# NEUROINFORMATICS-GROUP-FAV-KIV-ZCU/EEG_DataAnalysisPackage

Measured on AMD Instinct MI355X. Metric: epochs/sec feature-extracted (whole node) + % HBM roofline, 1/2/4/8 GPUs, higher is better.
Workload: dtype f64

## Files before the change

eeg_dataanalysispackage_amd/csrc/launch.h:

```cpp
#pragma once

#include <hip/hip_runtime_api.h>

#include <cstdint>

#include "guard.h"

namespace eegfx {

constexpr int kMaxChannels = 64;

struct ChanSel {
  int32_t col[kMaxChannels];
  float res[kMaxChannels];
};

hipError_t launch_cut_epochs(hipStream_t st, const void* raw, int fmt, int64_t n_frames, int ct,
                             const ChanSel& sel, int C, const int64_t* pos, int64_t n,
                             double* out, void* scratch, int* err);
hipError_t launch_cut_epochs(hipStream_t st, const void* raw, int fmt, int64_t n_frames, int ct,
                             const ChanSel& sel, int C, const int64_t* pos, int64_t n,
                             float* out, void* scratch, int* err);
bool cut_features_supported(int fmt, int ct, int C, const void* raw, const double* out,
                            const double* feat);
hipError_t launch_cut_features(hipStream_t st, const void* raw, int fmt, int64_t n_frames, int ct,
                               const ChanSel& sel, int C, const int64_t* pos, int64_t n,
                               double* out, double* feat, bool fast, void* scratch, int* err,
                               const Guard& guard);
bool cut_features_supported(int fmt, int ct, int C, const void* raw, const float* out,
                            const double* feat);
hipError_t launch_cut_features(hipStream_t st, const void* raw, int fmt, int64_t n_frames, int ct,
                               const ChanSel& sel, int C, const int64_t* pos, int64_t n,
                               float* out, double* feat, bool fast, void* scratch, int* err,
                               const Guard& guard);
hipError_t launch_features_from_epochs(hipStream_t st, const double* ep, int64_t n, int C, int skip,
                                       int nfeat, bool fast, double* out, int row_stride,
                                       const Guard& guard);
hipError_t launch_features_from_epochs(hipStream_t st, const float* ep, int64_t n, int C, int skip,
                                       int nfeat, bool fast, double* out, int row_stride,
                                       const Guard& guard);
hipError_t launch_narrow_epochs(hipStream_t st, const double* in, float* out, int64_t count);
bool features_small_supported(int C);
struct MailboxCmd {
  uint64_t req;
  uint32_t done;
  uint32_t stop;
  uint32_t alive;
  uint32_t pad_;
  const double* rows;
  double* out;
};
inline uint64_t mailbox_request(uint32_t seq, int C, int nfeat, int64_t n) {
  return (uint64_t)seq << 32 | (uint64_t)(C - 1) << 26 | (uint64_t)(nfeat - 1) << 21 |
         (uint64_t)n;
}
hipError_t launch_features_mailbox(hipStream_t st, MailboxCmd* mb, uint64_t idle_ticks,
                                   uint32_t gen);
hipError_t launch_features_small(hipStream_t st, const double* rows, int64_t n, int C, int nfeat,
                                 double* out);
hipError_t launch_synth(hipStream_t st, int16_t* dst, int64_t n_frames, int ct, uint64_t seed);

bool streaming_reads(int64_t n_frames, int64_t n, int64_t min_spacing);

bool fused_supported(int fmt, int ct, int C, const double* out);
size_t fused_scratch_bytes(int64_t n, int C);
hipError_t launch_fused_baseline(hipStream_t st, const void* raw, int64_t n_frames, int ct,
                                 const ChanSel& sel, int C, const int64_t* pos, int64_t n,
                                 void* scratch, int* err, int* guard_count,
                                 const Guard* guard = nullptr);
hipError_t launch_fused_window(hipStream_t st, const void* raw, int64_t n_frames, int ct,
                               const ChanSel& sel, int C, const int64_t* pos, int64_t n, bool fast,
                               const void* scratch, double* out, const Guard& guard,
                               bool track = false);
int64_t fused_window_bytes_per_epoch(int ct, int C);

bool wide_supported(int fmt, int ct, int C);
bool baseline_any_supported(int fmt, int ct, int C);
hipError_t launch_baseline_any(hipStream_t st, const void* raw, int fmt, int64_t n_frames, int ct,
                               const ChanSel& sel, int C, const int64_t* pos, int64_t n,
                               void* scratch, int* err, int* guard_count,
                               const Guard* guard = nullptr);
hipError_t launch_window_wide(hipStream_t st, const void* raw, int fmt, int64_t n_frames, int ct,
                              const ChanSel& sel, int C, const int64_t* pos, int64_t n, bool fast,
                              const void* scratch, double* out, const Guard& guard,
                              bool track = false);

hipError_t launch_pyramid_from_epochs(hipStream_t st, const double* ep, int64_t n, int C, int skip,
                                      int nfeat, double* out, int row_stride);
hipError_t launch_pyramid_from_epochs(hipStream_t st, const float* ep, int64_t n, int C, int skip,
                                      int nfeat, double* out, int row_stride);

hipError_t launch_guard_fixup_raw(hipStream_t st, const void* raw, int fmt, int64_t n_frames,
                                  int ct, const ChanSel& sel, int C, const int64_t* pos,
                                  const void* scratch, const Guard& g, double* out);

struct LrState {
  int32_t iter;
  int32_t converged;
  int32_t updates;
  int32_t pad;
  double w[];
};
constexpr int kLrMaxFeatures = 1024;

struct PlanResult {
  int64_t selected;
  int64_t balance;
  int64_t first_unparsable;
};
size_t plan_scratch_bytes(int64_t n);
hipError_t launch_plan_markers(hipStream_t st, const int64_t* pos, const int32_t* stim, int64_t n,
                               int64_t n_frames, int32_t guessed, int d0, void* scratch,
                               int64_t* pos_out, double* label_out, PlanResult* result);
int lr_grid(int64_t n);
hipError_t launch_lr_validate(hipStream_t st, const double* y, int64_t n, LrState* state);
constexpr int kGradLogistic = 0;
constexpr int kGradHinge = 1;
hipError_t launch_lr_iteration(hipStream_t st, int grad, const double* X, const double* y,
                               int64_t n, int d, const uint32_t* mask, int64_t count,
                               LrState* state, double* partial, int G, double step_size,
                               double reg, double tol, int max_iter);
hipError_t launch_lr_predict(hipStream_t st, int grad, const double* X, int64_t n, int d,
                             const double* w, double intercept, double threshold,
                             int use_threshold, double* out);


struct DtDecision {
  int32_t feature;
  int32_t split;
  int32_t left, right;
};
struct DtNode {
  int32_t feature, left, right, pad;
  double threshold, predict;
};
constexpr int kDtMaxBins = 256;
constexpr int kDtLdsCounters = 32768;
hipError_t launch_dt_bin(hipStream_t st, const double* X, const double* y, int64_t n, int d,
                         int T, const int32_t* nthr, const double* thr, int32_t* flags,
                         uint8_t* bins, uint8_t* label, int32_t* slot);
hipError_t launch_dt_hist(hipStream_t st, const uint8_t* bins, const uint8_t* label,
                          const int32_t* slot, int64_t n, int d, int B, int g0, int g,
                          uint32_t* hist);
hipError_t launch_dt_route(hipStream_t st, const uint8_t* bins, int64_t n, int d,
                           const DtDecision* dec, int32_t* slot);
hipError_t launch_dt_gather(hipStream_t st, const double* X, int d, const int64_t* idx, int64_t m,
                            double* out);
hipError_t launch_dt_predict(hipStream_t st, const double* X, int64_t n, int d,
                             const DtNode* nodes, int n_nodes, double* out);

hipError_t launch_rf_init(hipStream_t st, const uint8_t* weight, int64_t n, int num_trees,
                          int32_t* slot);
hipError_t launch_rf_hist(hipStream_t st, const uint8_t* bins, const uint8_t* label,
                          const uint8_t* weight, const int32_t* slot, int64_t n, int d, int B,
                          int k, int s0, int g, const int32_t* trees, int nt, const int32_t* sub,
                          uint32_t* hist);
hipError_t launch_rf_route(hipStream_t st, const uint8_t* bins, int64_t n, int d,
                           const int32_t* trees, int nt, int s0, int g, const DtDecision* dec,
                           int32_t* slot);
hipError_t launch_rf_predict(hipStream_t st, const double* X, int64_t n, int d,
                             const DtNode* nodes, const int32_t* offsets, int num_trees,
                             double* out);

}
```

eeg_dataanalysispackage_amd/csrc/logreg.hip:

```cpp
#include <hip/hip_runtime.h>

#include <cstdint>
#include <cstdlib>

#include "launch.h"

namespace eegfx {
namespace dev {

constexpr int kLrWaves = 4;
#ifndef EEGFX_LR_UNROLL
#define EEGFX_LR_UNROLL 4
#endif

__device__ __forceinline__ double wave_sum(double v) {
#pragma unroll
  for (int off = 32; off > 0; off >>= 1) v += __shfl_xor(v, off, 64);
  return v;
}

template <int GRAD>
__device__ __forceinline__ double grad_mult(double margin, double y) {
  if constexpr (GRAD == 0) {
    return 1.0 / (1.0 + exp(-margin)) - y;
  } else {
    const double s = 2.0 * y - 1.0;
    return 1.0 > s * margin ? -s : 0.0;
  }
}

template <int GRAD>
__device__ __forceinline__ double axpy_row(double mult, double x, double acc) {
  if constexpr (GRAD == 0) {
    return __builtin_fma(mult, x, acc);
  } else {
    return mult != 0.0 ? __builtin_fma(mult, x, acc) : acc;
  }
}

__device__ __forceinline__ bool sampled(const uint32_t* __restrict__ mask, int64_t r) {
  return !mask || ((mask[r >> 5] >> (r & 31)) & 1u);
}

template <int KD, int GRAD>
__global__ __launch_bounds__(64 * kLrWaves) void lr_grad_kernel(
    const double* __restrict__ X, const double* __restrict__ y, int64_t n, int d,
    const uint32_t* __restrict__ mask, const LrState* __restrict__ st,
    double* __restrict__ partial) {
  if (st->converged) return;
  __shared__ double acc_s[kLrWaves][64 * KD];
  const int lane = threadIdx.x & 63, w = threadIdx.x >> 6;
  const double* wt = st->w;
  double wv[KD], acc[KD];
#pragma unroll
  for (int k = 0; k < KD; ++k) {
    const int f = lane + 64 * k;
    wv[k] = f < d ? wt[f] : 0.0;
    acc[k] = 0.0;
  }
  const int64_t stride = (int64_t)gridDim.x * kLrWaves;
  for (int64_t r = (int64_t)blockIdx.x * kLrWaves + w; r < n; r += stride) {
    if (!sampled(mask, r)) continue;
    const double* row = X + r * d;
    double x[KD];
    double dot = 0.0;
#pragma unroll
    for (int k = 0; k < KD; ++k) {
      const int f = lane + 64 * k;
      x[k] = f < d ? row[f] : 0.0;
      dot = __builtin_fma(x[k], wv[k], dot);
    }
    dot = wave_sum(dot);
    const double mult = grad_mult<GRAD>(dot, y[r]);
#pragma unroll
    for (int k = 0; k < KD; ++k) acc[k] = axpy_row<GRAD>(mult, x[k], acc[k]);
  }
#pragma unroll
  for (int k = 0; k < KD; ++k) acc_s[w][lane + 64 * k] = acc[k];
  __syncthreads();
  for (int f = threadIdx.x; f < d; f += blockDim.x) {
    double s = acc_s[0][f];
#pragma unroll
    for (int v = 1; v < kLrWaves; ++v) s += acc_s[v][f];
    partial[(int64_t)blockIdx.x * d + f] = s;
  }
}

template <int CTRL>
__device__ __forceinline__ double dpp_d(double v) {
  const uint64_t u = __builtin_bit_cast(uint64_t, v);
  const int lo = __builtin_amdgcn_update_dpp(0, (int)(uint32_t)u, CTRL, 0xF, 0xF, false);
  const int hi = __builtin_amdgcn_update_dpp(0, (int)(uint32_t)(u >> 32), CTRL, 0xF, 0xF, false);
  return __builtin_bit_cast(double, ((uint64_t)(uint32_t)hi << 32) | (uint32_t)lo);
}
__device__ __forceinline__ double row16_sum(double v) {
  v += dpp_d<0xB1>(v);
  v += dpp_d<0x4E>(v);
  v += dpp_d<0x141>(v);
  v += dpp_d<0x140>(v);
  return v;
}

template <int FPL, int GRAD>
__global__ __launch_bounds__(64 * kLrWaves) void lr_grad16_kernel(
    const double* __restrict__ X, const double* __restrict__ y, int64_t n, int d,
    const uint32_t* __restrict__ mask, const LrState* __restrict__ st,
    double* __restrict__ partial) {
  if (st->converged) return;
  __shared__ double acc_s[kLrWaves * 4][16 * FPL];
  const int lane = threadIdx.x & 63, w = threadIdx.x >> 6;
  const int q = lane >> 4, j = lane & 15;
  double wv[FPL], acc[FPL];
#pragma unroll
  for (int k = 0; k < FPL; ++k) {
    const int f = j + 16 * k;
    wv[k] = f < d ? st->w[f] : 0.0;
    acc[k] = 0.0;
  }
  constexpr int U = EEGFX_LR_UNROLL;
  const int64_t stride = (int64_t)gridDim.x * kLrWaves * 4 * U;
  for (int64_t r0 = ((int64_t)blockIdx.x * kLrWaves + w) * 4 * U; r0 < n; r0 += stride) {
    double x[U][FPL], dot[U], yy[U];
#pragma unroll
    for (int u = 0; u < U; ++u) {
      const int64_t r = r0 + 4 * u + q;
      dot[u] = 0.0;
      if constexpr (GRAD == 0) {
        const bool ok = r < n && sampled(mask, r);
        const double* row = X + (ok ? r : 0) * d;
#pragma unroll
        for (int k = 0; k < FPL; ++k) {
          const int f = j + 16 * k;
          x[u][k] = (ok && f < d) ? row[f] : 0.0;
          dot[u] = __builtin_fma(x[u][k], wv[k], dot[u]);
        }
        yy[u] = ok ? y[r] : 0.0;
      } else {
        const double* row = X + (r < n ? r : n - 1) * d;
#pragma unroll
        for (int k = 0; k < FPL; ++k) {
          const int f = j + 16 * k;
          x[u][k] = row[f < d ? f : d - 1];
          dot[u] = __builtin_fma(x[u][k], wv[k], dot[u]);
        }
        yy[u] = y[r < n ? r : n - 1];
      }
    }
    double mult[U], msum = 0.0;
#pragma unroll
    for (int u = 0; u < U; ++u) {
      const double m = row16_sum(dot[u]);
      const bool ok = r0 + 4 * u + q < n && sampled(mask, r0 + 4 * u + q);
      mult[u] = ok ? grad_mult<GRAD>(m, yy[u]) : 0.0;
      msum += m;
    }
    if constexpr (GRAD == 1) {
      if (__builtin_amdgcn_ballot_w64(!(__builtin_fabs(msum) <= __DBL_MAX__)) != 0) {
#pragma unroll
        for (int u = 0; u < U; ++u) {
          double dt = 0.0;
#pragma unroll
          for (int k = 0; k < FPL; ++k) {
            if (j + 16 * k >= d) x[u][k] = 0.0;
            dt = __builtin_fma(x[u][k], wv[k], dt);
          }
          const double m = row16_sum(dt);
          const bool ok = r0 + 4 * u + q < n && sampled(mask, r0 + 4 * u + q);
          const double mu = ok ? grad_mult<GRAD>(m, yy[u]) : 0.0;
#pragma unroll
          for (int k = 0; k < FPL; ++k) acc[k] = axpy_row<GRAD>(mu, x[u][k], acc[k]);
        }
        continue;
      }
    }
#pragma unroll
    for (int u = 0; u < U; ++u) {
#pragma unroll
      for (int k = 0; k < FPL; ++k) acc[k] = __builtin_fma(mult[u], x[u][k], acc[k]);
    }
  }
#pragma unroll
  for (int k = 0; k < FPL; ++k) acc_s[w * 4 + q][j + 16 * k] = acc[k];
  __syncthreads();
  for (int f = threadIdx.x; f < d; f += blockDim.x) {
    double s = acc_s[0][f];
#pragma unroll
    for (int v = 1; v < kLrWaves * 4; ++v) s += acc_s[v][f];
    partial[(int64_t)blockIdx.x * d + f] = s;
  }
}

__global__ __launch_bounds__(256) void lr_update_kernel(const double* __restrict__ partial, int G,
                                                        int64_t n, int d, double step_size,
                                                        double reg, double tol, int max_iter,
                                                        LrState* __restrict__ st) {
  if (st->converged) return;
  __shared__ double red[2][256];
  __shared__ double gs[256];
  const int it = st->iter + 1;
  const double step = step_size / sqrt((double)it);
  const int K = d <= 128 ? (int)blockDim.x / d : 1;
  if (K > 1) {
    const int t = threadIdx.x, jj = t / d, f = t - jj * d;
    if (jj < K) {
      double a0 = 0.0, a1 = 0.0;
      int b = jj;
      for (; b + K < G; b += 2 * K) {
        a0 += partial[(int64_t)b * d + f];
        a1 += partial[(int64_t)(b + K) * d + f];
      }
      if (b < G) a0 += partial[(int64_t)b * d + f];
      gs[t] = a0 + a1;
    }
    __syncthreads();
  }
  double diff2 = 0.0, norm2 = 0.0;
  for (int f = threadIdx.x; f < d; f += blockDim.x) {
    double g = 0.0;
    if (K > 1) {
      for (int jj = 0; jj < K; ++jj) g += gs[jj * d + f];
    } else {
      for (int b = 0; b < G; ++b) g += partial[(int64_t)b * d + f];
    }
    g = g / (double)n;
    const double old = st->w[f];
    double nw = old * (1.0 - step * reg);
    nw = nw + (-step) * g;
    st->w[f] = nw;
    diff2 += (old - nw) * (old - nw);
    norm2 += nw * nw;
  }
  red[0][threadIdx.x] = diff2;
  red[1][threadIdx.x] = norm2;
  __syncthreads();
  for (int s = 128; s > 0; s >>= 1) {
    if ((int)threadIdx.x < s) {
      red[0][threadIdx.x] += red[0][threadIdx.x + s];
      red[1][threadIdx.x] += red[1][threadIdx.x + s];
    }
    __syncthreads();
  }
  if (threadIdx.x == 0) {
    st->iter = it;
    const int up = st->updates + 1;
    st->updates = up;
    const double diff = sqrt(red[0][0]), nrm = sqrt(red[1][0]);
    if ((up >= 2 && diff < tol * (nrm > 1.0 ? nrm : 1.0)) || it >= max_iter) st->converged = 1;
  }
}

__global__ void lr_skip_kernel(int max_iter, LrState* __restrict__ st) {
  if (st->converged || threadIdx.x != 0) return;
  st->iter += 1;
  if (st->iter >= max_iter) st->converged = 1;
}

template <int KD, int KIND>
__global__ __launch_bounds__(256) void lr_predict_kernel(const double* __restrict__ X, int64_t n,
                                                         int d, const double* __restrict__ wt,
                                                         double intercept, double threshold,
                                                         int use_threshold,
                                                         double* __restrict__ out) {
  const int lane = threadIdx.x & 63;
  const int64_t r = (int64_t)blockIdx.x * 4 + (threadIdx.x >> 6);
  if (r >= n) return;
  double dot = 0.0;
#pragma unroll
  for (int k = 0; k < KD; ++k) {
    const int f = lane + 64 * k;
    if (f < d) dot = __builtin_fma(X[r * d + f], wt[f], dot);
  }
  dot = wave_sum(dot);
  if (lane == 0) {
    const double margin = dot + intercept;
    const double score = KIND == 0 ? 1.0 / (1.0 + exp(-margin)) : margin;
    out[r] = use_threshold ? (score > threshold ? 1.0 : 0.0) : score;
  }
}

__global__ __launch_bounds__(256) void lr_validate_kernel(const double* __restrict__ y, int64_t n,
                                                          LrState* __restrict__ st) {
  for (int64_t i = (int64_t)blockIdx.x * blockDim.x + threadIdx.x; i < n;
       i += (int64_t)gridDim.x * blockDim.x)
    if (!(y[i] == 0.0 || y[i] == 1.0)) st->converged = 2;
}

}

hipError_t launch_lr_validate(hipStream_t st, const double* y, int64_t n, LrState* state) {
  const int64_t g = (n + 255) / 256;
  hipLaunchKernelGGL(dev::lr_validate_kernel, dim3((unsigned)(g < 1 ? 1 : (g > 4096 ? 4096 : g))),
                     dim3(256), 0, st, y, n, state);
  return hipGetLastError();
}

int lr_grid(int64_t n) {
  constexpr int64_t cap = 512;
  const int64_t g = (n + 16 * dev::kLrWaves - 1) / (16 * dev::kLrWaves);
  return (int)(g < 1 ? 1 : (g > cap ? cap : g));
}

#define EEGFX_LR_KD(KD, CALL) \
  case KD:                    \
    CALL;                     \
    break;

template <int GRAD>
static hipError_t lr_iteration(hipStream_t st, const double* X, const double* y, int64_t n, int d,
                               const uint32_t* mask, int64_t count, LrState* state,
                               double* partial, int G, double step_size, double reg, double tol,
                               int max_iter) {
  if (count == 0) {
    hipLaunchKernelGGL(dev::lr_skip_kernel, dim3(1), dim3(64), 0, st, max_iter, state);
    return hipGetLastError();
  }
  if (d <= 128) {
    const int fpl = (d + 15) / 16;
    switch (fpl <= 1 ? 1 : fpl <= 2 ? 2 : fpl <= 3 ? 3 : fpl <= 4 ? 4 : 8) {
      EEGFX_LR_KD(1, hipLaunchKernelGGL((dev::lr_grad16_kernel<1, GRAD>), dim3(G), dim3(256), 0,
                                        st, X, y, n, d, mask, state, partial))
      EEGFX_LR_KD(2, hipLaunchKernelGGL((dev::lr_grad16_kernel<2, GRAD>), dim3(G), dim3(256), 0,
                                        st, X, y, n, d, mask, state, partial))
      EEGFX_LR_KD(3, hipLaunchKernelGGL((dev::lr_grad16_kernel<3, GRAD>), dim3(G), dim3(256), 0,
                                        st, X, y, n, d, mask, state, partial))
      EEGFX_LR_KD(4, hipLaunchKernelGGL((dev::lr_grad16_kernel<4, GRAD>), dim3(G), dim3(256), 0,
                                        st, X, y, n, d, mask, state, partial))
      EEGFX_LR_KD(8, hipLaunchKernelGGL((dev::lr_grad16_kernel<8, GRAD>), dim3(G), dim3(256), 0,
                                        st, X, y, n, d, mask, state, partial))
    }
  } else {
    const int kd = (d + 63) / 64;
    switch (kd <= 1 ? 1 : kd <= 2 ? 2 : kd <= 4 ? 4 : kd <= 8 ? 8 : 16) {
      EEGFX_LR_KD(1, hipLaunchKernelGGL((dev::lr_grad_kernel<1, GRAD>), dim3(G), dim3(256), 0, st,
                                        X, y, n, d, mask, state, partial))
      EEGFX_LR_KD(2, hipLaunchKernelGGL((dev::lr_grad_kernel<2, GRAD>), dim3(G), dim3(256), 0, st,
                                        X, y, n, d, mask, state, partial))
      EEGFX_LR_KD(4, hipLaunchKernelGGL((dev::lr_grad_kernel<4, GRAD>), dim3(G), dim3(256), 0, st,
                                        X, y, n, d, mask, state, partial))
      EEGFX_LR_KD(8, hipLaunchKernelGGL((dev::lr_grad_kernel<8, GRAD>), dim3(G), dim3(256), 0, st,
                                        X, y, n, d, mask, state, partial))
      EEGFX_LR_KD(16, hipLaunchKernelGGL((dev::lr_grad_kernel<16, GRAD>), dim3(G), dim3(256), 0,
                                         st, X, y, n, d, mask, state, partial))
    }
  }
  hipLaunchKernelGGL(dev::lr_update_kernel, dim3(1), dim3(256), 0, st, partial, G, count, d,
                     step_size, reg, tol, max_iter, state);
  return hipGetLastError();
}

hipError_t launch_lr_iteration(hipStream_t st, int grad, const double* X, const double* y,
                               int64_t n, int d, const uint32_t* mask, int64_t count,
                               LrState* state, double* partial, int G, double step_size,
                               double reg, double tol, int max_iter) {
  return grad == kGradHinge ? lr_iteration<1>(st, X, y, n, d, mask, count, state, partial, G,
                                              step_size, reg, tol, max_iter)
                            : lr_iteration<0>(st, X, y, n, d, mask, count, state, partial, G,
                                              step_size, reg, tol, max_iter);
}

template <int KIND>
static hipError_t lr_predict(hipStream_t st, const double* X, int64_t n, int d, const double* w,
                             double intercept, double threshold, int use_threshold, double* out) {
  const dim3 grid((unsigned)((n + 3) / 4));
  const int kd = (d + 63) / 64;
  switch (kd <= 1 ? 1 : kd <= 2 ? 2 : kd <= 4 ? 4 : kd <= 8 ? 8 : 16) {
    EEGFX_LR_KD(1, hipLaunchKernelGGL((dev::lr_predict_kernel<1, KIND>), grid, dim3(256), 0, st, X,
                                      n, d, w, intercept, threshold, use_threshold, out))
    EEGFX_LR_KD(2, hipLaunchKernelGGL((dev::lr_predict_kernel<2, KIND>), grid, dim3(256), 0, st, X,
                                      n, d, w, intercept, threshold, use_threshold, out))
    EEGFX_LR_KD(4, hipLaunchKernelGGL((dev::lr_predict_kernel<4, KIND>), grid, dim3(256), 0, st, X,
                                      n, d, w, intercept, threshold, use_threshold, out))
    EEGFX_LR_KD(8, hipLaunchKernelGGL((dev::lr_predict_kernel<8, KIND>), grid, dim3(256), 0, st, X,
                                      n, d, w, intercept, threshold, use_threshold, out))
    EEGFX_LR_KD(16, hipLaunchKernelGGL((dev::lr_predict_kernel<16, KIND>), grid, dim3(256), 0, st,
                                       X, n, d, w, intercept, threshold, use_threshold, out))
  }
  return hipGetLastError();
}

hipError_t launch_lr_predict(hipStream_t st, int grad, const double* X, int64_t n, int d,
                             const double* w, double intercept, double threshold,
                             int use_threshold, double* out) {
  if (n == 0) return hipSuccess;
  return grad == kGradHinge
             ? lr_predict<1>(st, X, n, d, w, intercept, threshold, use_threshold, out)
             : lr_predict<0>(st, X, n, d, w, intercept, threshold, use_threshold, out);
}
#undef EEGFX_LR_KD

}
```

eeg_dataanalysispackage_amd/csrc/lds_dma.h:

```cpp
#pragma once

#include <hip/hip_runtime.h>

#include <cstdint>

namespace eegfx {
namespace dev {

typedef __attribute__((address_space(3))) void* lds_ptr_t;

#ifndef EEGFX_DMA_POLICY
#define EEGFX_DMA_POLICY ""
#endif

template <bool NT = false>
__device__ __forceinline__ void dma16_s(const uint8_t* sbase, uint32_t voff, const void* lds_dst) {
  const uint32_t lds = (uint32_t)(uintptr_t)(lds_ptr_t)lds_dst;
  uint32_t saved;
  if constexpr (NT) {
    asm volatile(
        "s_mov_b32 %0, m0\n\t"
        "s_mov_b32 m0, %1\n\t"
        "s_nop 0\n\t"
        "global_load_lds_dwordx4 %2, %3 nt\n\t"
        "s_nop 0\n\t"
        "s_mov_b32 m0, %0"
        : "=&s"(saved)
        : "s"(lds), "v"(voff), "s"(sbase)
        : "memory");
  } else {
    asm volatile(
        "s_mov_b32 %0, m0\n\t"
        "s_mov_b32 m0, %1\n\t"
        "s_nop 0\n\t"
        "global_load_lds_dwordx4 %2, %3" EEGFX_DMA_POLICY "\n\t"
        "s_nop 0\n\t"
        "s_mov_b32 m0, %0"
        : "=&s"(saved)
        : "s"(lds), "v"(voff), "s"(sbase)
        : "memory");
  }
}

__device__ __forceinline__ void dma_drain() { asm volatile("s_waitcnt vmcnt(0)" ::: "memory"); }

}
}
```

Before: 1.189 billion.

## Fuse logistic-regression update into gradient kernel via last-block-arrives ticket

Removes the separate single-block lr_update_kernel launch per iteration. Each gradient block now stores its partial sum atomically and takes a ticket on a counter in LrState, and the last block to arrive performs the reduction and weight update. The partial reduction loop is also batched so more loads are in flight. This saves one kernel launch and one dependency per iteration, at the cost of device-scope atomics and fences, and it requires the repurposed pad field to start at zero.

```diff
diff --git a/eeg_dataanalysispackage_amd/csrc/launch.h b/eeg_dataanalysispackage_amd/csrc/launch.h
--- a/eeg_dataanalysispackage_amd/csrc/launch.h
+++ b/eeg_dataanalysispackage_amd/csrc/launch.h
@@ -98,7 +98,7 @@
   int32_t iter;
   int32_t converged;
   int32_t updates;
-  int32_t pad;
+  int32_t arrived;
   double w[];
 };
 constexpr int kLrMaxFeatures = 1024;
diff --git a/eeg_dataanalysispackage_amd/csrc/logreg.hip b/eeg_dataanalysispackage_amd/csrc/logreg.hip
--- a/eeg_dataanalysispackage_amd/csrc/logreg.hip
+++ b/eeg_dataanalysispackage_amd/csrc/logreg.hip
@@ -42,159 +42,34 @@
   return !mask || ((mask[r >> 5] >> (r & 31)) & 1u);
 }
 
-template <int KD, int GRAD>
-__global__ __launch_bounds__(64 * kLrWaves) void lr_grad_kernel(
-    const double* __restrict__ X, const double* __restrict__ y, int64_t n, int d,
-    const uint32_t* __restrict__ mask, const LrState* __restrict__ st,
-    double* __restrict__ partial) {
-  if (st->converged) return;
-  __shared__ double acc_s[kLrWaves][64 * KD];
-  const int lane = threadIdx.x & 63, w = threadIdx.x >> 6;
-  const double* wt = st->w;
-  double wv[KD], acc[KD];
-#pragma unroll
-  for (int k = 0; k < KD; ++k) {
-    const int f = lane + 64 * k;
-    wv[k] = f < d ? wt[f] : 0.0;
-    acc[k] = 0.0;
-  }
-  const int64_t stride = (int64_t)gridDim.x * kLrWaves;
-  for (int64_t r = (int64_t)blockIdx.x * kLrWaves + w; r < n; r += stride) {
-    if (!sampled(mask, r)) continue;
-    const double* row = X + r * d;
-    double x[KD];
-    double dot = 0.0;
-#pragma unroll
-    for (int k = 0; k < KD; ++k) {
-      const int f = lane + 64 * k;
-      x[k] = f < d ? row[f] : 0.0;
-      dot = __builtin_fma(x[k], wv[k], dot);
-    }
-    dot = wave_sum(dot);
-    const double mult = grad_mult<GRAD>(dot, y[r]);
-#pragma unroll
-    for (int k = 0; k < KD; ++k) acc[k] = axpy_row<GRAD>(mult, x[k], acc[k]);
-  }
-#pragma unroll
-  for (int k = 0; k < KD; ++k) acc_s[w][lane + 64 * k] = acc[k];
+constexpr int kLrBatch = 16;
+
+__device__ __forceinline__ void store_partial(double* p, double v) {
+  __hip_atomic_store(p, v, __ATOMIC_RELAXED, __HIP_MEMORY_SCOPE_AGENT);
+}
+
+__device__ __forceinline__ bool lr_arrive_last(int32_t* arrived) {
+  __shared__ int last_s;
+  asm volatile("s_waitcnt vmcnt(0)" ::: "memory");
   __syncthreads();
-  for (int f = threadIdx.x; f < d; f += blockDim.x) {
-    double s = acc_s[0][f];
-#pragma unroll
-    for (int v = 1; v < kLrWaves; ++v) s += acc_s[v][f];
-    partial[(int64_t)blockIdx.x * d + f] = s;
-  }
-}
-
-template <int CTRL>
-__device__ __forceinline__ double dpp_d(double v) {
-  const uint64_t u = __builtin_bit_cast(uint64_t, v);
-  const int lo = __builtin_amdgcn_update_dpp(0, (int)(uint32_t)u, CTRL, 0xF, 0xF, false);
-  const int hi = __builtin_amdgcn_update_dpp(0, (int)(uint32_t)(u >> 32), CTRL, 0xF, 0xF, false);
-  return __builtin_bit_cast(double, ((uint64_t)(uint32_t)hi << 32) | (uint32_t)lo);
-}
-__device__ __forceinline__ double row16_sum(double v) {
-  v += dpp_d<0xB1>(v);
-  v += dpp_d<0x4E>(v);
-  v += dpp_d<0x141>(v);
-  v += dpp_d<0x140>(v);
-  return v;
-}
-
-template <int FPL, int GRAD>
-__global__ __launch_bounds__(64 * kLrWaves) void lr_grad16_kernel(
-    const double* __restrict__ X, const double* __restrict__ y, int64_t n, int d,
-    const uint32_t* __restrict__ mask, const LrState* __restrict__ st,
-    double* __restrict__ partial) {
-  if (st->converged) return;
-  __shared__ double acc_s[kLrWaves * 4][16 * FPL];
-  const int lane = threadIdx.x & 63, w = threadIdx.x >> 6;
-  const int q = lane >> 4, j = lane & 15;
-  double wv[FPL], acc[FPL];
-#pragma unroll
-  for (int k = 0; k < FPL; ++k) {
-    const int f = j + 16 * k;
-    wv[k] = f < d ? st->w[f] : 0.0;
-    acc[k] = 0.0;
-  }
-  constexpr int U = EEGFX_LR_UNROLL;
-  const int64_t stride = (int64_t)gridDim.x * kLrWaves * 4 * U;
-  for (int64_t r0 = ((int64_t)blockIdx.x * kLrWaves + w) * 4 * U; r0 < n; r0 += stride) {
-    double x[U][FPL], dot[U], yy[U];
-#pragma unroll
-    for (int u = 0; u < U; ++u) {
-      const int64_t r = r0 + 4 * u + q;
-      dot[u] = 0.0;
-      if constexpr (GRAD == 0) {
-        const bool ok = r < n && sampled(mask, r);
-        const double* row = X + (ok ? r : 0) * d;
-#pragma unroll
-        for (int k = 0; k < FPL; ++k) {
-          const int f = j + 16 * k;
-          x[u][k] = (ok && f < d) ? row[f] : 0.0;
-          dot[u] = __builtin_fma(x[u][k], wv[k], dot[u]);
-        }
-        yy[u] = ok ? y[r] : 0.0;
-      } else {
-        const double* row = X + (r < n ? r : n - 1) * d;
-#pragma unroll
-        for (int k = 0; k < FPL; ++k) {
-          const int f = j + 16 * k;
-          x[u][k] = row[f < d ? f : d - 1];
-          dot[u] = __builtin_fma(x[u][k], wv[k], dot[u]);
-        }
-        yy[u] = y[r < n ? r : n - 1];
-      }
-    }
-    double mult[U], msum = 0.0;
-#pragma unroll
-    for (int u = 0; u < U; ++u) {
-      const double m = row16_sum(dot[u]);
-      const bool ok = r0 + 4 * u + q < n && sampled(mask, r0 + 4 * u + q);
-      mult[u] = ok ? grad_mult<GRAD>(m, yy[u]) : 0.0;
-      msum += m;
-    }
-    if constexpr (GRAD == 1) {
-      if (__builtin_amdgcn_ballot_w64(!(__builtin_fabs(msum) <= __DBL_MAX__)) != 0) {
-#pragma unroll
-        for (int u = 0; u < U; ++u) {
-          double dt = 0.0;
-#pragma unroll
-          for (int k = 0; k < FPL; ++k) {
-            if (j + 16 * k >= d) x[u][k] = 0.0;
-            dt = __builtin_fma(x[u][k], wv[k], dt);
-          }
-          const double m = row16_sum(dt);
-          const bool ok = r0 + 4 * u + q < n && sampled(mask, r0 + 4 * u + q);
-          const double mu = ok ? grad_mult<GRAD>(m, yy[u]) : 0.0;
-#pragma unroll
-          for (int k = 0; k < FPL; ++k) acc[k] = axpy_row<GRAD>(mu, x[u][k], acc[k]);
-        }
-        continue;
-      }
-    }
-#pragma unroll
-    for (int u = 0; u < U; ++u) {
-#pragma unroll
-      for (int k = 0; k < FPL; ++k) acc[k] = __builtin_fma(mult[u], x[u][k], acc[k]);
-    }
-  }
-#pragma unroll
-  for (int k = 0; k < FPL; ++k) acc_s[w * 4 + q][j + 16 * k] = acc[k];
+  if (threadIdx.x == 0) {
+    const int ticket =
+        __hip_atomic_fetch_add(arrived, 1, __ATOMIC_RELAXED, __HIP_MEMORY_SCOPE_AGENT);
+    const int last = ticket == (int)gridDim.x - 1;
+    if (last) {
+      __hip_atomic_store(arrived, 0, __ATOMIC_RELAXED, __HIP_MEMORY_SCOPE_AGENT);
+      __builtin_amdgcn_fence(__ATOMIC_ACQUIRE, "agent");
+      asm volatile("s_waitcnt vmcnt(0)" ::: "memory");
+    }
+    last_s = last;
+  }
   __syncthreads();
-  for (int f = threadIdx.x; f < d; f += blockDim.x) {
-    double s = acc_s[0][f];
-#pragma unroll
-    for (int v = 1; v < kLrWaves * 4; ++v) s += acc_s[v][f];
-    partial[(int64_t)blockIdx.x * d + f] = s;
-  }
-}
-
-__global__ __launch_bounds__(256) void lr_update_kernel(const double* __restrict__ partial, int G,
-                                                        int64_t n, int d, double step_size,
-                                                        double reg, double tol, int max_iter,
-                                                        LrState* __restrict__ st) {
-  if (st->converged) return;
+  return last_s != 0;
+}
+
+__device__ __forceinline__ void lr_update(const double* partial, int G, int64_t count, int d,
+                                          double step_size, double reg, double tol, int max_iter,
+                                          LrState* st) {
   __shared__ double red[2][256];
   __shared__ double gs[256];
   const int it = st->iter + 1;
@@ -204,12 +79,20 @@
     const int t = threadIdx.x, jj = t / d, f = t - jj * d;
     if (jj < K) {
       double a0 = 0.0, a1 = 0.0;
-      int b = jj;
-      for (; b + K < G; b += 2 * K) {
-        a0 += partial[(int64_t)b * d + f];
-        a1 += partial[(int64_t)(b + K) * d + f];
+      for (int b = jj; b < G; b += 2 * kLrBatch * K) {
+        double v0[kLrBatch], v1[kLrBatch];
+#pragma unroll
+        for (int i = 0; i < kLrBatch; ++i) {
+          const int b0 = b + 2 * i * K, b1 = b0 + K;
+          v0[i] = partial[(int64_t)(b0 < G ? b0 : G - 1) * d + f];
+          v1[i] = partial[(int64_t)(b1 < G ? b1 : G - 1) * d + f];
+        }
+#pragma unroll
+        for (int i = 0; i < kLrBatch; ++i) {
+          if (b + 2 * i * K < G) a0 += v0[i];
+          if (b + (2 * i + 1) * K < G) a1 += v1[i];
+        }
       }
-      if (b < G) a0 += partial[(int64_t)b * d + f];
       gs[t] = a0 + a1;
     }
     __syncthreads();
@@ -220,9 +103,17 @@
     if (K > 1) {
       for (int jj = 0; jj < K; ++jj) g += gs[jj * d + f];
     } else {
-      for (int b = 0; b < G; ++b) g += partial[(int64_t)b * d + f];
-    }
-    g = g / (double)n;
+      for (int b = 0; b < G; b += 2 * kLrBatch) {
+        double v[2 * kLrBatch];
+#pragma unroll
+        for (int i = 0; i < 2 * kLrBatch; ++i)
+          v[i] = partial[(int64_t)(b + i < G ? b + i : G - 1) * d + f];
+#pragma unroll
+        for (int i = 0; i < 2 * kLrBatch; ++i)
+          if (b + i < G) g += v[i];
+      }
+    }
+    g = g / (double)count;
     const double old = st->w[f];
     double nw = old * (1.0 - step * reg);
     nw = nw + (-step) * g;
@@ -247,6 +138,158 @@
     const double diff = sqrt(red[0][0]), nrm = sqrt(red[1][0]);
     if ((up >= 2 && diff < tol * (nrm > 1.0 ? nrm : 1.0)) || it >= max_iter) st->converged = 1;
   }
+}
+
+template <int KD, int GRAD>
+__global__ __launch_bounds__(64 * kLrWaves) void lr_grad_kernel(
+    const double* __restrict__ X, const double* __restrict__ y, int64_t n, int d,
+    const uint32_t* __restrict__ mask, int64_t count, double step_size, double reg, double tol,
+    int max_iter, LrState* __restrict__ st, double* __restrict__ partial) {
+  if (st->converged) return;
+  __shared__ double acc_s[kLrWaves][64 * KD];
+  const int lane = threadIdx.x & 63, w = threadIdx.x >> 6;
+  const double* wt = st->w;
+  double wv[KD], acc[KD];
+#pragma unroll
+  for (int k = 0; k < KD; ++k) {
+    const int f = lane + 64 * k;
+    wv[k] = f < d ? wt[f] : 0.0;
+    acc[k] = 0.0;
+  }
+  const int64_t stride = (int64_t)gridDim.x * kLrWaves;
+  for (int64_t r = (int64_t)blockIdx.x * kLrWaves + w; r < n; r += stride) {
+    if (!sampled(mask, r)) continue;
+    const double* row = X + r * d;
+    double x[KD];
+    double dot = 0.0;
+#pragma unroll
+    for (int k = 0; k < KD; ++k) {
+      const int f = lane + 64 * k;
+      x[k] = f < d ? row[f] : 0.0;
+      dot = __builtin_fma(x[k], wv[k], dot);
+    }
+    dot = wave_sum(dot);
+    const double mult = grad_mult<GRAD>(dot, y[r]);
+#pragma unroll
+    for (int k = 0; k < KD; ++k) acc[k] = axpy_row<GRAD>(mult, x[k], acc[k]);
+  }
+#pragma unroll
+  for (int k = 0; k < KD; ++k) acc_s[w][lane + 64 * k] = acc[k];
+  __syncthreads();
+  for (int f = threadIdx.x; f < d; f += blockDim.x) {
+    double s = acc_s[0][f];
+#pragma unroll
+    for (int v = 1; v < kLrWaves; ++v) s += acc_s[v][f];
+    store_partial(&partial[(int64_t)blockIdx.x * d + f], s);
+  }
+  if (lr_arrive_last(&st->arrived))
+    lr_update(partial, (int)gridDim.x, count, d, step_size, reg, tol, max_iter, st);
+}
+
+template <int CTRL>
+__device__ __forceinline__ double dpp_d(double v) {
+  const uint64_t u = __builtin_bit_cast(uint64_t, v);
+  const int lo = __builtin_amdgcn_update_dpp(0, (int)(uint32_t)u, CTRL, 0xF, 0xF, false);
+  const int hi = __builtin_amdgcn_update_dpp(0, (int)(uint32_t)(u >> 32), CTRL, 0xF, 0xF, false);
+  return __builtin_bit_cast(double, ((uint64_t)(uint32_t)hi << 32) | (uint32_t)lo);
+}
+__device__ __forceinline__ double row16_sum(double v) {
+  v += dpp_d<0xB1>(v);
+  v += dpp_d<0x4E>(v);
+  v += dpp_d<0x141>(v);
+  v += dpp_d<0x140>(v);
+  return v;
+}
+
+template <int FPL, int GRAD>
+__global__ __launch_bounds__(64 * kLrWaves) void lr_grad16_kernel(
+    const double* __restrict__ X, const double* __restrict__ y, int64_t n, int d,
+    const uint32_t* __restrict__ mask, int64_t count, double step_size, double reg, double tol,
+    int max_iter, LrState* __restrict__ st, double* __restrict__ partial) {
+  if (st->converged) return;
+  __shared__ double acc_s[kLrWaves * 4][16 * FPL];
+  const int lane = threadIdx.x & 63, w = threadIdx.x >> 6;
+  const int q = lane >> 4, j = lane & 15;
+  double wv[FPL], acc[FPL];
+#pragma unroll
+  for (int k = 0; k < FPL; ++k) {
+    const int f = j + 16 * k;
+    wv[k] = f < d ? st->w[f] : 0.0;
+    acc[k] = 0.0;
+  }
+  constexpr int U = EEGFX_LR_UNROLL;
+  const int64_t stride = (int64_t)gridDim.x * kLrWaves * 4 * U;
+  for (int64_t r0 = ((int64_t)blockIdx.x * kLrWaves + w) * 4 * U; r0 < n; r0 += stride) {
+    double x[U][FPL], dot[U], yy[U];
+#pragma unroll
+    for (int u = 0; u < U; ++u) {
+      const int64_t r = r0 + 4 * u + q;
+      dot[u] = 0.0;
+      if constexpr (GRAD == 0) {
+        const bool ok = r < n && sampled(mask, r);
+        const double* row = X + (ok ? r : 0) * d;
+#pragma unroll
+        for (int k = 0; k < FPL; ++k) {
+          const int f = j + 16 * k;
+          x[u][k] = (ok && f < d) ? row[f] : 0.0;
+          dot[u] = __builtin_fma(x[u][k], wv[k], dot[u]);
+        }
+        yy[u] = ok ? y[r] : 0.0;
+      } else {
+        const double* row = X + (r < n ? r : n - 1) * d;
+#pragma unroll
+        for (int k = 0; k < FPL; ++k) {
+          const int f = j + 16 * k;
+          x[u][k] = row[f < d ? f : d - 1];
+          dot[u] = __builtin_fma(x[u][k], wv[k], dot[u]);
+        }
+        yy[u] = y[r < n ? r : n - 1];
+      }
+    }
+    double mult[U], msum = 0.0;
+#pragma unroll
+    for (int u = 0; u < U; ++u) {
+      const double m = row16_sum(dot[u]);
+      const bool ok = r0 + 4 * u + q < n && sampled(mask, r0 + 4 * u + q);
+      mult[u] = ok ? grad_mult<GRAD>(m, yy[u]) : 0.0;
+      msum += m;
+    }
+    if constexpr (GRAD == 1) {
+      if (__builtin_amdgcn_ballot_w64(!(__builtin_fabs(msum) <= __DBL_MAX__)) != 0) {
+#pragma unroll
+        for (int u = 0; u < U; ++u) {
+          double dt = 0.0;
+#pragma unroll
+          for (int k = 0; k < FPL; ++k) {
+            if (j + 16 * k >= d) x[u][k] = 0.0;
+            dt = __builtin_fma(x[u][k], wv[k], dt);
+          }
+          const double m = row16_sum(dt);
+          const bool ok = r0 + 4 * u + q < n && sampled(mask, r0 + 4 * u + q);
+          const double mu = ok ? grad_mult<GRAD>(m, yy[u]) : 0.0;
+#pragma unroll
+          for (int k = 0; k < FPL; ++k) acc[k] = axpy_row<GRAD>(mu, x[u][k], acc[k]);
+        }
+        continue;
+      }
+    }
+#pragma unroll
+    for (int u = 0; u < U; ++u) {
+#pragma unroll
+      for (int k = 0; k < FPL; ++k) acc[k] = __builtin_fma(mult[u], x[u][k], acc[k]);
+    }
+  }
+#pragma unroll
+  for (int k = 0; k < FPL; ++k) acc_s[w * 4 + q][j + 16 * k] = acc[k];
+  __syncthreads();
+  for (int f = threadIdx.x; f < d; f += blockDim.x) {
+    double s = acc_s[0][f];
+#pragma unroll
+    for (int v = 1; v < kLrWaves * 4; ++v) s += acc_s[v][f];
+    store_partial(&partial[(int64_t)blockIdx.x * d + f], s);
+  }
+  if (lr_arrive_last(&st->arrived))
+    lr_update(partial, (int)gridDim.x, count, d, step_size, reg, tol, max_iter, st);
 }
 
 __global__ void lr_skip_kernel(int max_iter, LrState* __restrict__ st) {
@@ -314,37 +357,30 @@
     hipLaunchKernelGGL(dev::lr_skip_kernel, dim3(1), dim3(64), 0, st, max_iter, state);
     return hipGetLastError();
   }
+#define EEGFX_LR_GRAD(KERNEL, KD)                                                               \
+  EEGFX_LR_KD(KD, hipLaunchKernelGGL((dev::KERNEL<KD, GRAD>), dim3(G), dim3(256), 0, st, X, y, n, \
+                                     d, mask, count, step_size, reg, tol, max_iter, state,        \
+                                     partial))
   if (d <= 128) {
     const int fpl = (d + 15) / 16;
     switch (fpl <= 1 ? 1 : fpl <= 2 ? 2 : fpl <= 3 ? 3 : fpl <= 4 ? 4 : 8) {
-      EEGFX_LR_KD(1, hipLaunchKernelGGL((dev::lr_grad16_kernel<1, GRAD>), dim3(G), dim3(256), 0,
-                                        st, X, y, n, d, mask, state, partial))
-      EEGFX_LR_KD(2, hipLaunchKernelGGL((dev::lr_grad16_kernel<2, GRAD>), dim3(G), dim3(256), 0,
-                                        st, X, y, n, d, mask, state, partial))
-      EEGFX_LR_KD(3, hipLaunchKernelGGL((dev::lr_grad16_kernel<3, GRAD>), dim3(G), dim3(256), 0,
-                                        st, X, y, n, d, mask, state, partial))
-      EEGFX_LR_KD(4, hipLaunchKernelGGL((dev::lr_grad16_kernel<4, GRAD>), dim3(G), dim3(256), 0,
-                                        st, X, y, n, d, mask, state, partial))
-      EEGFX_LR_KD(8, hipLaunchKernelGGL((dev::lr_grad16_kernel<8, GRAD>), dim3(G), dim3(256), 0,
-                                        st, X, y, n, d, mask, state, partial))
+      EEGFX_LR_GRAD(lr_grad16_kernel, 1)
+      EEGFX_LR_GRAD(lr_grad16_kernel, 2)
+      EEGFX_LR_GRAD(lr_grad16_kernel, 3)
+      EEGFX_LR_GRAD(lr_grad16_kernel, 4)
+      EEGFX_LR_GRAD(lr_grad16_kernel, 8)
     }
   } else {
     const int kd = (d + 63) / 64;
     switch (kd <= 1 ? 1 : kd <= 2 ? 2 : kd <= 4 ? 4 : kd <= 8 ? 8 : 16) {
-      EEGFX_LR_KD(1, hipLaunchKernelGGL((dev::lr_grad_kernel<1, GRAD>), dim3(G), dim3(256), 0, st,
-                                        X, y, n, d, mask, state, partial))
-      EEGFX_LR_KD(2, hipLaunchKernelGGL((dev::lr_grad_kernel<2, GRAD>), dim3(G), dim3(256), 0, st,
-                                        X, y, n, d, mask, state, partial))
-      EEGFX_LR_KD(4, hipLaunchKernelGGL((dev::lr_grad_kernel<4, GRAD>), dim3(G), dim3(256), 0, st,
-                                        X, y, n, d, mask, state, partial))
-      EEGFX_LR_KD(8, hipLaunchKernelGGL((dev::lr_grad_kernel<8, GRAD>), dim3(G), dim3(256), 0, st,
-                                        X, y, n, d, mask, state, partial))
-      EEGFX_LR_KD(16, hipLaunchKernelGGL((dev::lr_grad_kernel<16, GRAD>), dim3(G), dim3(256), 0,
-                                         st, X, y, n, d, mask, state, partial))
-    }
-  }
-  hipLaunchKernelGGL(dev::lr_update_kernel, dim3(1), dim3(256), 0, st, partial, G, count, d,
-                     step_size, reg, tol, max_iter, state);
+      EEGFX_LR_GRAD(lr_grad_kernel, 1)
+      EEGFX_LR_GRAD(lr_grad_kernel, 2)
+      EEGFX_LR_GRAD(lr_grad_kernel, 4)
+      EEGFX_LR_GRAD(lr_grad_kernel, 8)
+      EEGFX_LR_GRAD(lr_grad_kernel, 16)
+    }
+  }
+#undef EEGFX_LR_GRAD
   return hipGetLastError();
 }
 
```

Result: no change. 1.183 billion (-0.5%).

## Stream logistic-regression rows through a per-wave LDS DMA ring buffer

Applied to the files above, without the earlier changes.

Adds a new gradient kernel for the unmasked logistic (GRAD==0) case with d<=128 and 16-byte aligned X. Each wave prefetches several row tiles of X and y ahead into an LDS ring using global_load_lds DMA with the nt hint, and waits on vmcnt counters before consuming each stage. The aim is to hide HBM latency with deeper in-flight loads. The update kernel's reduction over per-block partials is also unrolled into batched loads for more memory-level parallelism. The ring uses a large LDS allocation, which may lower occupancy, and the hand-counted vmcnt bookkeeping is fragile.

```diff
diff --git a/eeg_dataanalysispackage_amd/csrc/lds_dma.h b/eeg_dataanalysispackage_amd/csrc/lds_dma.h
--- a/eeg_dataanalysispackage_amd/csrc/lds_dma.h
+++ b/eeg_dataanalysispackage_amd/csrc/lds_dma.h
@@ -42,7 +42,57 @@
   }
 }
 
+template <bool NT = false>
+__device__ __forceinline__ void dma4_s(const uint8_t* sbase, uint32_t voff, const void* lds_dst) {
+  const uint32_t lds = (uint32_t)(uintptr_t)(lds_ptr_t)lds_dst;
+  uint32_t saved;
+  if constexpr (NT) {
+    asm volatile(
+        "s_mov_b32 %0, m0\n\t"
+        "s_mov_b32 m0, %1\n\t"
+        "s_nop 0\n\t"
+        "global_load_lds_dword %2, %3 nt\n\t"
+        "s_nop 0\n\t"
+        "s_mov_b32 m0, %0"
+        : "=&s"(saved)
+        : "s"(lds), "v"(voff), "s"(sbase)
+        : "memory");
+  } else {
+    asm volatile(
+        "s_mov_b32 %0, m0\n\t"
+        "s_mov_b32 m0, %1\n\t"
+        "s_nop 0\n\t"
+        "global_load_lds_dword %2, %3\n\t"
+        "s_nop 0\n\t"
+        "s_mov_b32 m0, %0"
+        : "=&s"(saved)
+        : "s"(lds), "v"(voff), "s"(sbase)
+        : "memory");
+  }
+}
+
 __device__ __forceinline__ void dma_drain() { asm volatile("s_waitcnt vmcnt(0)" ::: "memory"); }
+
+__device__ __forceinline__ void dma_wait(int k) {
+#define EEGFX_VMCNT(N) \
+  case N:              \
+    asm volatile("s_waitcnt vmcnt(" #N ")" ::: "memory"); \
+    break;
+  switch (k) {
+    EEGFX_VMCNT(1) EEGFX_VMCNT(2) EEGFX_VMCNT(3) EEGFX_VMCNT(4) EEGFX_VMCNT(5) EEGFX_VMCNT(6)
+    EEGFX_VMCNT(7) EEGFX_VMCNT(8) EEGFX_VMCNT(9) EEGFX_VMCNT(10) EEGFX_VMCNT(11) EEGFX_VMCNT(12)
+    EEGFX_VMCNT(13) EEGFX_VMCNT(14) EEGFX_VMCNT(15) EEGFX_VMCNT(16) EEGFX_VMCNT(17)
+    EEGFX_VMCNT(18) EEGFX_VMCNT(19) EEGFX_VMCNT(20) EEGFX_VMCNT(21) EEGFX_VMCNT(22)
+    EEGFX_VMCNT(23) EEGFX_VMCNT(24)
+    default:
+      asm volatile("s_waitcnt vmcnt(0)" ::: "memory");
+  }
+#undef EEGFX_VMCNT
+}
+
+__device__ __forceinline__ void lds_reads_done() {
+  asm volatile("s_waitcnt lgkmcnt(0)" ::: "memory");
+}
 
 }
 }
diff --git a/eeg_dataanalysispackage_amd/csrc/logreg.hip b/eeg_dataanalysispackage_amd/csrc/logreg.hip
--- a/eeg_dataanalysispackage_amd/csrc/logreg.hip
+++ b/eeg_dataanalysispackage_amd/csrc/logreg.hip
@@ -4,11 +4,13 @@
 #include <cstdlib>
 
 #include "launch.h"
+#include "lds_dma.h"
 
 namespace eegfx {
 namespace dev {
 
 constexpr int kLrWaves = 4;
+constexpr int kLrAhead = 16;
 #ifndef EEGFX_LR_UNROLL
 #define EEGFX_LR_UNROLL 4
 #endif
@@ -179,6 +181,134 @@
       for (int k = 0; k < FPL; ++k) acc[k] = __builtin_fma(mult[u], x[u][k], acc[k]);
     }
   }
+#pragma unroll
+  for (int k = 0; k < FPL; ++k) acc_s[w * 4 + q][j + 16 * k] = acc[k];
+  __syncthreads();
+  for (int f = threadIdx.x; f < d; f += blockDim.x) {
+    double s = acc_s[0][f];
+#pragma unroll
+    for (int v = 1; v < kLrWaves * 4; ++v) s += acc_s[v][f];
+    partial[(int64_t)blockIdx.x * d + f] = s;
+  }
+}
+
+template <int FPL>
+struct LrRing {
+  static constexpr int SUB = FPL <= 3 ? 4 : 1;
+  static constexpr int S = FPL == 1 ? 8 : FPL == 2 ? 4 : FPL == 3 ? 3 : FPL == 4 ? 8 : 4;
+  static constexpr int XB = 4 * SUB * 16 * FPL * 8;
+  static constexpr int STG = XB + 128;
+  static constexpr int LDS = kLrWaves * S * STG;
+  static_assert(STG % 16 == 0, "a DMA lands on 16-byte quads");
+  static_assert(2 * LDS <= 160 * 1024, "2 workgroups per CU share the 160 KB of LDS");
+  static_assert(LDS >= kLrWaves * 4 * 16 * FPL * 8, "acc_s reuses the ring");
+  static_assert((S - 1) * ((XB >> 10) + 1) <= 24, "dma_wait's table");
+};
+
+constexpr bool kLrRingNt = true;
+
+template <int FPL>
+__global__ __launch_bounds__(64 * kLrWaves) void lr_grad16_ring_kernel(
+    const double* __restrict__ X, const double* __restrict__ y, int64_t n, int d,
+    const LrState* __restrict__ st, double* __restrict__ partial) {
+  if (st->converged) return;
+  using R = LrRing<FPL>;
+  constexpr int SUB = R::SUB, S = R::S, TPG = 4 / SUB;
+  __shared__ __attribute__((aligned(16))) uint8_t ring[R::LDS];
+  const int lane = threadIdx.x & 63, w = __builtin_amdgcn_readfirstlane(threadIdx.x >> 6);
+  const int q = lane >> 4, j = lane & 15;
+  double wv[FPL], acc[FPL];
+#pragma unroll
+  for (int k = 0; k < FPL; ++k) {
+    const int f = j + 16 * k;
+    wv[k] = f < d ? st->w[f] : 0.0;
+    acc[k] = 0.0;
+  }
+#pragma unroll
+  for (int k = 0; k < FPL; ++k) asm volatile("" : "+v"(wv[k]));
+
+  uint8_t* mine = ring + w * (S * R::STG);
+  const int xb = 32 * SUB * d;
+  const int ni = ((xb + 1023) >> 10) + 1;
+  const int64_t nb = n * d * 8;
+  const int64_t stride = (int64_t)gridDim.x * kLrWaves * 16;
+  const int64_t row_w = ((int64_t)blockIdx.x * kLrWaves + w) * 16;
+  auto first = [&](int t) { return row_w + (int64_t)(t / TPG) * stride + (t % TPG) * (4 * SUB); };
+  int T = 0, TF = 0;
+  if (row_w < n) {
+    const int64_t pf = n - row_w >= 16 ? (n - 16 - row_w) / stride + 1 : 0;
+    const int64_t rest = n - (row_w + pf * stride);
+    const int64_t rc = rest < 0 ? 0 : rest > 16 ? 16 : rest;
+    TF = (int)(pf * TPG + rc / (4 * SUB));
+    T = (int)(pf * TPG + (rc + 4 * SUB - 1) / (4 * SUB));
+  }
+  auto issue = [&](int t) {
+    const int64_t fr = first(t);
+    uint8_t* dst = mine + (t % S) * R::STG;
+    const uint8_t* sx = (const uint8_t*)X + fr * d * 8;
+    const uint8_t* sy = (const uint8_t*)y + fr * 8;
+    if (t < TF) {
+      for (int p = 0; p < ni - 1; ++p) {
+        const uint32_t off = 1024u * p + 16u * lane;
+        if (off < (uint32_t)xb) dma16_s<kLrRingNt>(sx, off, dst + 1024 * p);
+      }
+      if (lane < 8 * SUB) dma4_s<kLrRingNt>(sy, 4u * lane, dst + R::XB);
+    } else {
+      const int64_t left = nb - fr * d * 8;
+      for (int p = 0; 1024 * p < left; ++p) {
+        const uint32_t off = 1024u * p + 16u * lane;
+        if ((int64_t)off + 16 <= left) dma16_s<kLrRingNt>(sx, off, dst + 1024 * p);
+      }
+      if (left & 8) {
+        const uint32_t o = (uint32_t)(left - 8);
+        if (lane < 2) dma4_s<kLrRingNt>(sx, o + 4u * lane, dst + o);
+      }
+      if (4 * lane + 4 <= (n - fr) * 8) dma4_s<kLrRingNt>(sy, 4u * lane, dst + R::XB);
+    }
+  };
+
+  for (int t = 0; t < S - 1 && t < T; ++t) issue(t);
+  for (int t = 0; t < T; ++t) {
+    if (t + S - 1 < T) {
+      lds_reads_done();
+      issue(t + S - 1);
+    }
+    const int later = TF - 1 - t;
+    dma_wait((later < 0 ? 0 : later > S - 1 ? S - 1 : later) * ni);
+
+    const int64_t fr = first(t);
+    const uint8_t* stg = mine + (t % S) * R::STG;
+    const double* xs = (const double*)stg;
+    const double* ys = (const double*)(stg + R::XB);
+    double x[SUB][FPL], dot[SUB], yy[SUB];
+#pragma unroll
+    for (int u = 0; u < SUB; ++u) {
+      const bool ok = fr + 4 * u + q < n;
+      const double* row = xs + (4 * u + q) * d;
+      dot[u] = 0.0;
+#pragma unroll
+      for (int k = 0; k < FPL; ++k) {
+        const int f = j + 16 * k;
+        x[u][k] = (ok && f < d) ? row[f] : 0.0;
+        dot[u] = __builtin_fma(x[u][k], wv[k], dot[u]);
+      }
+      yy[u] = ok ? ys[4 * u + q] : 0.0;
+    }
+    double mult[SUB];
+#pragma unroll
+    for (int u = 0; u < SUB; ++u) {
+      const double m = row16_sum(dot[u]);
+      mult[u] = fr + 4 * u + q < n ? grad_mult<0>(m, yy[u]) : 0.0;
+    }
+#pragma unroll
+    for (int u = 0; u < SUB; ++u) {
+#pragma unroll
+      for (int k = 0; k < FPL; ++k) acc[k] = __builtin_fma(mult[u], x[u][k], acc[k]);
+    }
+  }
+  dma_drain();
+  __syncthreads();
+  double(*acc_s)[16 * FPL] = (double(*)[16 * FPL])ring;
 #pragma unroll
   for (int k = 0; k < FPL; ++k) acc_s[w * 4 + q][j + 16 * k] = acc[k];
   __syncthreads();
@@ -205,6 +335,16 @@
     if (jj < K) {
       double a0 = 0.0, a1 = 0.0;
       int b = jj;
+      for (; b + (2 * kLrAhead - 1) * K < G; b += 2 * kLrAhead * K) {
+        double v[2 * kLrAhead];
+#pragma unroll
+        for (int i = 0; i < 2 * kLrAhead; ++i) v[i] = partial[(int64_t)(b + i * K) * d + f];
+#pragma unroll
+        for (int i = 0; i < kLrAhead; ++i) {
+          a0 += v[2 * i];
+          a1 += v[2 * i + 1];
+        }
+      }
       for (; b + K < G; b += 2 * K) {
         a0 += partial[(int64_t)b * d + f];
         a1 += partial[(int64_t)(b + K) * d + f];
@@ -220,7 +360,15 @@
     if (K > 1) {
       for (int jj = 0; jj < K; ++jj) g += gs[jj * d + f];
     } else {
-      for (int b = 0; b < G; ++b) g += partial[(int64_t)b * d + f];
+      int b = 0;
+      for (; b + 2 * kLrAhead <= G; b += 2 * kLrAhead) {
+        double v[2 * kLrAhead];
+#pragma unroll
+        for (int i = 0; i < 2 * kLrAhead; ++i) v[i] = partial[(int64_t)(b + i) * d + f];
+#pragma unroll
+        for (int i = 0; i < 2 * kLrAhead; ++i) g += v[i];
+      }
+      for (; b < G; ++b) g += partial[(int64_t)b * d + f];
     }
     g = g / (double)n;
     const double old = st->w[f];
@@ -300,6 +448,10 @@
   return (int)(g < 1 ? 1 : (g > cap ? cap : g));
 }
 
+static bool lr_ring_supported(int grad, const double* X, int d, const uint32_t* mask) {
+  return grad == 0 && !mask && d <= 128 && ((uintptr_t)X & 15) == 0;
+}
+
 #define EEGFX_LR_KD(KD, CALL) \
   case KD:                    \
     CALL;                     \
@@ -314,7 +466,21 @@
     hipLaunchKernelGGL(dev::lr_skip_kernel, dim3(1), dim3(64), 0, st, max_iter, state);
     return hipGetLastError();
   }
-  if (d <= 128) {
+  if (lr_ring_supported(GRAD, X, d, mask)) {
+    const int fpl = (d + 15) / 16;
+    switch (fpl <= 1 ? 1 : fpl <= 2 ? 2 : fpl <= 3 ? 3 : fpl <= 4 ? 4 : 8) {
+      EEGFX_LR_KD(1, hipLaunchKernelGGL((dev::lr_grad16_ring_kernel<1>), dim3(G), dim3(256), 0,
+                                        st, X, y, n, d, state, partial))
+      EEGFX_LR_KD(2, hipLaunchKernelGGL((dev::lr_grad16_ring_kernel<2>), dim3(G), dim3(256), 0,
+                                        st, X, y, n, d, state, partial))
+      EEGFX_LR_KD(3, hipLaunchKernelGGL((dev::lr_grad16_ring_kernel<3>), dim3(G), dim3(256), 0,
+                                        st, X, y, n, d, state, partial))
+      EEGFX_LR_KD(4, hipLaunchKernelGGL((dev::lr_grad16_ring_kernel<4>), dim3(G), dim3(256), 0,
+                                        st, X, y, n, d, state, partial))
+      EEGFX_LR_KD(8, hipLaunchKernelGGL((dev::lr_grad16_ring_kernel<8>), dim3(G), dim3(256), 0,
+                                        st, X, y, n, d, state, partial))
+    }
+  } else if (d <= 128) {
     const int fpl = (d + 15) / 16;
     switch (fpl <= 1 ? 1 : fpl <= 2 ? 2 : fpl <= 3 ? 3 : fpl <= 4 ? 4 : 8) {
       EEGFX_LR_KD(1, hipLaunchKernelGGL((dev::lr_grad16_kernel<1, GRAD>), dim3(G), dim3(256), 0,
```

After: 1.154 billion before, 1.153 billion after. About the same (-0.1%).
